# fengranMark/HAConvDR

Hardware: AMD Instinct MI355X
Metric: queries/sec (encode+top-100) over N-passage 768-d corpus; HBM GB/s vs peak (higher is better)
Workload: dtype bf16 MFMA operands with fp32 accumulate / LayerNorm / softmax in the encoder (cosine vs the fp32 reference within 1e-3, measured ~1e-5); search scores and order = the fp32 fmaf chain, bit-exact

## Files before the change

### haconvdr_amd/csrc/encoder.hip

```cpp
#include <type_traits>
#include "hac_common.h"

#include <cmath>
#include <cstring>
#include <map>
#include <string>
#include <vector>

namespace hac {
namespace {

typedef __bf16 bf16;
typedef __bf16 bf16x8 __attribute__((ext_vector_type(8)));
typedef __bf16 bf16x4 __attribute__((ext_vector_type(4)));
typedef float f32x16 __attribute__((ext_vector_type(16)));
typedef float f32x4 __attribute__((ext_vector_type(4)));
typedef float f4v __attribute__((ext_vector_type(4)));

constexpr int H = 768;
constexpr int NH = 12;
constexpr int DH = 64;
constexpr int FF = 3072;
constexpr int SEQ_ALIGN = 32;
constexpr int MT = 256, BK = 64;
// ... 1193 lines not shown
    if (i < n) dst[i] = (bf16)src[i];
}

}
}

using namespace hac;

namespace {

inline int pad_len(int L) { return (L + SEQ_ALIGN - 1) / SEQ_ALIGN * SEQ_ALIGN; }

struct LayerW {
    bf16 *wqkv = nullptr, *wo = nullptr, *w1 = nullptr, *w2 = nullptr;
    float *bqkv = nullptr, *bo = nullptr, *b1 = nullptr, *b2 = nullptr;
    float *ln1g = nullptr, *ln1b = nullptr, *ln2g = nullptr, *ln2b = nullptr;
    bf16 *wqkv8 = nullptr, *w18 = nullptr;
    float *fold = nullptr;
    bf16 *wqkv_lo = nullptr, *wo_lo = nullptr, *w1_lo = nullptr, *w2_lo = nullptr;
};
void free_layer(LayerW &l) {
    for (void *p : std::initializer_list<void *>{l.wqkv, l.wo, l.w1, l.w2, l.wqkv8, l.w18, l.wqkv_lo, l.wo_lo, l.w1_lo, l.w2_lo, l.bqkv, l.fold})
        if (p) (void)hipFree(p);
    l = LayerW();
}
struct Plan {
    const char *gemm = "none";
    int sub_batches = 0;
    long rows = 0;
    const char *graph = "off";
    int precision = 0, pooling = 0, model = 0;
    int ks_out = 1, ks_down = 1;
    int attn_pipe = 0;
};

}

struct hac_encoder {
    hac_encoder_config cfg;
    int device = 0;
    hipStream_t stream = nullptr;
    std::map<std::string, float *> raw;
    std::map<std::string, size_t> raw_count;
    std::vector<LayerW> layers;
    float *word = nullptr, *posw = nullptr, *typew = nullptr, *embg = nullptr, *embb = nullptr;
    float *wh = nullptr, *bh = nullptr, *ng = nullptr, *nb = nullptr;
    bool finalized = false;
    GrowBuf ws_x, ws_xb, ws_q, ws_k, ws_vt, ws_ctx, ws_y, ws_h, ws_seq, ws_ids, ws_mask, ws_out, ws_cls, ws_stats;
    GrowBuf ws_ksplit;
    GrowBuf ws_yb, ws_part, ws_idstats;
    size_t idstats_rows = 0;
    int precision = 0;
    bool split_weights = false;
    int model = 0;
    int pooling = 0;
    GrowBuf ws_pool;
    GrowBuf ws_xb_lo, ws_q_lo, ws_k_lo, ws_vt_lo, ws_ctx_lo, ws_h_lo, ws_cls_lo;
    int attn_mode = 0;
    int attn_pipe = -1;
    int gemm_mode = -1;
    int attn_qsplit = -1;
    int g8_stagger = -1;
    void *h_pin = nullptr;
    size_t h_pin_bytes = 0;
    int *h_len = nullptr;
    size_t h_len_cap = 0;
    unsigned prof_mask = 0;
    struct EvPool {
        std::vector<std::pair<hipEvent_t, hipEvent_t>> ev;
        size_t used = 0;
    } pools[1 + HAC_ENC_NCLASS];
    long max_tokens = 524288;
    int n_cu = 256;
    Plan plan;
    char last_plan[160] = "none";
    int graph_mode = -1;
    int attn_qs_pin = 0;
    int ks_pin_out = 0, ks_pin_down = 0;
    int ksplit_mode = -1;
    struct GraphEntry {
        hipGraph_t graph = nullptr;
        hipGraphExec_t exec = nullptr;
        uint64_t sig = 0;
        int seen = 0;
        Plan plan;
    };
    std::map<uint64_t, GraphEntry> graphs;
    hipEvent_t graph_done = nullptr;
    bool graph_done_armed = false;
    GrowBuf ws_gids, ws_gmask, ws_gout;
    GrowBuf ws_dump;
    GrowBuf ws_identgb;
    GrowBuf ws_redo;
    int *h_redo = nullptr;
    hipEvent_t redo_ev = nullptr;
    bool redo_pending = false;
    long redo_items = 0;
    unsigned pipe_skip_mask = 0;
    unsigned forwards_since_retry = 0;
    GrowBuf ws_clk;
    bool clk_valid = false;
    hipEvent_t clk_ev = nullptr;
};

namespace {

int enc_fail_missing(const std::string &name) { return fail(HAC_ERR_INVALID, "encoder weight '%s' was never set", name.c_str()); }

// ... 101 lines not shown
    };
    for (int i = 0; i < e->cfg.n_layers; ++i) {
        const std::string q = std::string(model_prefix(e)) + "encoder.layer." + std::to_string(i) + ".";
        LayerW &l = e->layers[i];
        float *t;
        if (!l.wqkv_lo) HAC_HIP(hipMalloc((void **)&l.wqkv_lo, (size_t)3 * H * H * sizeof(bf16)));
        if (!l.wo_lo) HAC_HIP(hipMalloc((void **)&l.wo_lo, (size_t)H * H * sizeof(bf16)));
        if (!l.w1_lo) HAC_HIP(hipMalloc((void **)&l.w1_lo, (size_t)FF * H * sizeof(bf16)));
        if (!l.w2_lo) HAC_HIP(hipMalloc((void **)&l.w2_lo, (size_t)H * FF * sizeof(bf16)));
        const char *qkv[3] = {"attention.self.query.weight", "attention.self.key.weight", "attention.self.value.weight"};
        for (int j = 0; j < 3; ++j) {
            HAC_TRY(get_raw(e, q + qkv[j], (size_t)H * H, &t));
            lo(t, (size_t)H * H, l.wqkv_lo + (size_t)j * H * H);
        }
        HAC_TRY(get_raw(e, q + "attention.output.dense.weight", (size_t)H * H, &t));
        lo(t, (size_t)H * H, l.wo_lo);
        HAC_TRY(get_raw(e, q + "intermediate.dense.weight", (size_t)FF * H, &t));
        lo(t, (size_t)FF * H, l.w1_lo);
        HAC_TRY(get_raw(e, q + "output.dense.weight", (size_t)H * FF, &t));
        lo(t, (size_t)H * FF, l.w2_lo);
        HAC_HIP(hipGetLastError());
    }
    HAC_HIP(hipStreamSynchronize(e->stream));
    e->split_weights = true;
    return HAC_OK;
}
int begin_call(hac_encoder *e) {
    e->plan.sub_batches = 0;
    e->plan.rows = 0;
    e->plan.graph = "off";
    e->plan.precision = e->precision;
    e->plan.pooling = e->pooling;
    e->plan.model = e->model;
    return e->precision == 1 ? ensure_split_weights(e) : HAC_OK;
}

struct Fwd {
    int B, L, L32;
    long Mp, Mc;
    SeqInfo s;
    const int *total;
    int family;
    bool big, mean;
    hipStream_t st;
    float *x, *y;
    float2 *statsA, *statsF;
    bf16 *xb, *q, *k, *vt, *ctx, *h;
    bf16 *xb_lo, *q_lo, *k_lo, *vt_lo, *ctx_lo, *h_lo;
    bf16 *yAb;
    float2 *part, *idstats;
    int ks_out, ks_down;
    float *kpart;
    size_t part_stride;
    bf16 *ctx_c, *xb_c, *h_c, *ctx_c_lo, *xb_c_lo, *h_c_lo;
    float *x_c, *y_c, *x2_c;
};

int pick_ksplit(int K, long Mp_plan, long wg_slots, int pin, int ksplit_mode) {
    if (wg_slots == 0 || ksplit_mode == 0) return 1;
    const int KT = K / 64, min_kt = KT >= 48 ? 8 : 4;
    if (pin > 0 && KT % pin == 0 && KT / pin >= 3) return pin;
    const long tiles = (Mp_plan / 128) * (H / 128);
    int S = 1;
    double best = KT * 0.6;
    for (int cand : {2, 3, 4, 6}) {
        if (KT % cand || KT / cand < min_kt || tiles * cand > wg_slots) continue;
// ... 249 lines not shown
int layer_gemm8(hac_encoder *e, const Fwd &f, int li) {
    const LayerW &w = e->layers[li];
    const PrevLN p = prev_ln(e, f, li);
    const hipStream_t st = f.st;
    Gemm8Args a{};
    HAC_TRY(qkv_gemm8(e, f, li, false, a));
    HAC_TRY(attention(e, f, li, false));
    a.A = f.ctx; a.W = w.wo; a.N = H; a.K = H; a.cvec = w.bo; a.resid = f.xb; a.yb = f.yAb; a.part = f.part;
    a.rstats = li ? p.stats : f.idstats;
    a.rgamma = li ? p.g : (const float *)e->ws_identgb.p;
    a.rbeta = li ? p.b : (const float *)e->ws_identgb.p + H;
    a.stagger = stagger8(e, f, H, 0, 8);
    HAC_PROFILED(e, st, HAC_ENC_CLASS_OUTPROJ, launch_gemm8<EPI8_RESID>(e, a, st));
    a.stagger = 0;
    HAC_PROFILED(e, st, HAC_ENC_CLASS_LN, ln_combine_kernel<<<dim3((unsigned)(f.Mp / 256)), dim3(256), 0, st>>>(f.part, H / 64, H, f.total, e->cfg.ln_eps, f.statsA));
    a.A = f.yAb; a.astats = f.statsA; a.W = w.w18; a.N = FF; a.K = H; a.wsum = w.fold + 6 * H; a.cvec = w.fold + 6 * H + FF; a.h = f.h;
    a.n_groups = 2;
    if (e->prof_mask >> 1) {
        HAC_TRY(e->ws_clk.reserve(32));
        a.clk = (unsigned long long *)e->ws_clk.p;
        e->clk_valid = true;
    }
    HAC_TRY(prof_begin(e, 1 + HAC_ENC_CLASS_FFN_UP, st));
    launch_gemm8<EPI8_GELU>(e, a, st);
    if (a.clk) {
        if (!e->clk_ev) HAC_HIP(hipEventCreateWithFlags(&e->clk_ev, hipEventDisableTiming));
        HAC_HIP(hipEventRecord(e->clk_ev, st));
    }
    a.clk = nullptr;
    HAC_TRY(prof_end(e, 1 + HAC_ENC_CLASS_FFN_UP, st));
    a.n_groups = 1;
    a.A = f.h; a.W = w.w2; a.N = H; a.K = FF; a.cvec = w.b2; a.resid = f.yAb; a.yb = f.xb;
    a.rstats = f.statsA; a.rgamma = w.ln1g; a.rbeta = w.ln1b;
    HAC_PROFILED(e, st, HAC_ENC_CLASS_FFN_DOWN, launch_gemm8<EPI8_RESID>(e, a, st));
    HAC_PROFILED(e, st, HAC_ENC_CLASS_LN, ln_combine_kernel<<<dim3((unsigned)(f.Mp / 256)), dim3(256), 0, st>>>(f.part, H / 64, H, f.total, e->cfg.ln_eps, f.statsF));
    return HAC_OK;
}

int tail_classic(hac_encoder *e, const Fwd &f, int li) {
    const LayerW &w = e->layers[li];
    const PrevLN p = prev_ln(e, f, li);
    const hipStream_t st = f.st;
    const bool g8 = f.family == FAM_GEMM8;
    GemmArgs g{};
    Gemm8Args a{};
    HAC_TRY(g8 ? qkv_gemm8(e, f, li, true, a) : qkv_classic(e, f, li, g));
    HAC_TRY(attention(e, f, li, true));
    gather_cls_kernel<<<dim3((unsigned)f.Mc), dim3(256), 0, st>>>(f.ctx, f.x, g8 ? f.xb : nullptr, p.stats, p.g, p.b, f.s, f.B, f.ctx_c, f.x_c);
    g.total_rows = f.s.nb;
    g.A = f.ctx_c; g.W = w.wo; g.bias = w.bo; g.N = H; g.K = H; g.resid = f.x_c; g.y = f.y_c; g.rstats = nullptr;
    launch_gemm128<EPI_RESID>(e, g, st);
    ln_rows_kernel<<<dim3((unsigned)(f.Mc / 4)), dim3(256), 0, st>>>(f.y_c, f.s.nb, w.ln1g, w.ln1b, e->cfg.ln_eps, f.x2_c, f.xb_c);
    g.A = f.xb_c; g.W = w.w1; g.bias = w.b1; g.N = FF; g.K = H; g.h = f.h_c;
    launch_gemm128<EPI_GELU>(e, g, st);
    g.A = f.h_c; g.W = w.w2; g.bias = w.b2; g.N = H; g.K = FF; g.resid = f.x2_c; g.y = f.y_c;
    launch_gemm128<EPI_RESID>(e, g, st);
    ln_rows_kernel<<<dim3((unsigned)(f.Mc / 4)), dim3(256), 0, st>>>(f.y_c, f.s.nb, w.ln2g, w.ln2b, e->cfg.ln_eps, f.x_c, f.xb_c);
    return HAC_OK;
}

template <int EPI>
void launch_gemm_split(const hac_encoder *e, const GemmSplitArgs &ga, hipStream_t st) {
    gemm_split_nt_kernel<EPI><<<dim3((unsigned)e->n_cu), dim3(256), SPLIT_GEMM_LDS, st>>>(ga);
}
int qkv_attention_split(hac_encoder *e, const Fwd &f, int li, bool last, GemmSplitArgs &ga) {
    const LayerW &w = e->layers[li];
    const hipStream_t st = f.st;
// ... 142 lines not shown
    if ((long)B * pad_len(L) > GRAPH_MAX_ROWS || (long)B * pad_len(L) > e->max_tokens) return false;
    hipStreamCaptureStatus cs = hipStreamCaptureStatusNone;
    if (hipStreamIsCapturing(st, &cs) != hipSuccess || cs != hipStreamCaptureStatusNone) return false;
    return true;
}
template <typename IT>
int graph_capture(hac_encoder *e, hac_encoder::GraphEntry &ge, const IT *gids, const IT *gmask, int B, int L, float *gout) {
    if (ge.exec) graphs_quiesce(e);
    if (ge.exec) (void)hipGraphExecDestroy(ge.exec);
    if (ge.graph) (void)hipGraphDestroy(ge.graph);
    ge.exec = nullptr;
    ge.graph = nullptr;
    HAC_HIP(hipStreamSynchronize(e->stream));
    HAC_HIP(hipStreamBeginCapture(e->stream, hipStreamCaptureModeThreadLocal));
    const int rc = run_forward<IT>(e, gids, gmask, B, L, gout, e->stream);
    const hipError_t ce = hipStreamEndCapture(e->stream, &ge.graph);
    if (rc != HAC_OK) return rc;
    if (ce != hipSuccess || !ge.graph) return fail(HAC_ERR_HIP, "hipStreamEndCapture failed: %s", hipGetErrorString(ce));
    HAC_HIP(hipGraphInstantiate(&ge.exec, ge.graph, nullptr, nullptr, 0));
    ge.sig = ws_signature(e);
    ge.plan = e->plan;
    return HAC_OK;
}
template <typename IT>
int forward_graph(hac_encoder *e, const IT *ids, const IT *mask, int B, int L, float *out_dev, hipStream_t st) {
    const size_t n_in = (size_t)B * L * sizeof(IT), n_out = (size_t)B * H * 4;
    HAC_TRY(e->ws_gids.reserve(n_in));
    HAC_TRY(e->ws_gmask.reserve(n_in));
    HAC_TRY(e->ws_gout.reserve(n_out));
    const uint64_t key = ((uint64_t)B << 40) | ((uint64_t)L << 24) | ((uint64_t)sizeof(IT) << 16) | ((uint64_t)(e->attn_mode & 1) << 8) |
                         ((uint64_t)((e->gemm_mode + 1) & 3) << 4) | ((uint64_t)(e->ksplit_mode & 1) << 12) |
                         ((uint64_t)(e->attn_qsplit & 1) << 13) | ((uint64_t)(e->g8_stagger & 1) << 14) | ((uint64_t)((e->attn_pipe + 1) & 3) << 15) |
                         ((uint64_t)(e->precision & 1) << 20) | ((uint64_t)(e->pooling & 1) << 21) |
                         ((uint64_t)(e->model & 1) << 22);
    if (e->graphs.size() >= GRAPH_MAX_SHAPES && e->graphs.find(key) == e->graphs.end()) drop_graphs(e);
    hac_encoder::GraphEntry &ge = e->graphs[key];
    const IT *gids = (const IT *)e->ws_gids.p, *gmask = (const IT *)e->ws_gmask.p;
    float *gout = (float *)e->ws_gout.p;
    HAC_HIP(hipMemcpyAsync(e->ws_gids.p, ids, n_in, hipMemcpyDeviceToDevice, st));
    HAC_HIP(hipMemcpyAsync(e->ws_gmask.p, mask, n_in, hipMemcpyDeviceToDevice, st));
    if (ge.seen == 0) {
        HAC_TRY(run_forward<IT>(e, gids, gmask, B, L, gout, st));
        ge.seen = 1;
        e->plan.graph = "eager-first";
    } else {
        if (!ge.exec || ge.sig != ws_signature(e)) HAC_TRY(graph_capture<IT>(e, ge, gids, gmask, B, L, gout));
        HAC_HIP(hipGraphLaunch(ge.exec, st));
        if (!e->graph_done) HAC_HIP(hipEventCreateWithFlags(&e->graph_done, hipEventDisableTiming));
        HAC_HIP(hipEventRecord(e->graph_done, st));
        e->graph_done_armed = true;
        e->plan = ge.plan;
        e->plan.graph = "replay";
    }
    HAC_HIP(hipMemcpyAsync(out_dev, gout, n_out, hipMemcpyDeviceToDevice, st));
    return HAC_OK;
}

template <typename IT>
int forward_batched(hac_encoder *e, const IT *ids, const IT *mask, int B, int L, float *out_dev, hipStream_t st) {
    const int L32 = pad_len(L);
    HAC_TRY(begin_call(e));
    if (graph_eligible(e, B, L, st)) return forward_graph<IT>(e, ids, mask, B, L, out_dev, st);
    if ((long)B * L32 <= e->max_tokens) return run_forward<IT>(e, ids, mask, B, L, out_dev, st);
    SeqInfo s;
    HAC_TRY(seq_layout(e, B, L, s));
    seq_prep_kernel<IT><<<dim3(B), dim3(512), 0, st>>>(ids, mask, L, s, e->cfg.pad_token_id, e->cfg.vocab, e->model == 1 ? POS_BERT : POS_ROBERTA);
    HAC_HIP(hipGetLastError());
// ... 62 lines not shown
    HAC_HIP(hipMalloc((void **)&l.w18, (size_t)FF * H * sizeof(bf16)));
    HAC_HIP(hipMalloc((void **)&l.fold, (size_t)(2 * 3 * H + 2 * FF) * 4));
    const float *pg = i ? e->layers[i - 1].ln2g : nullptr, *pb = i ? e->layers[i - 1].ln2b : nullptr;
    const float qscale = 0.125f * 1.44269504088896341f;
    for (int j = 0; j < 3; ++j)
        fold_ln_kernel<<<dim3(H), dim3(256), 0, e->stream>>>(ws[j], bs[j], pg, pb, H, j == 0 ? qscale : 1.0f, l.wqkv8 + (size_t)j * H * H,
                                                             l.fold + j * H, l.fold + 3 * H + j * H);
    HAC_TRY(get_raw(e, q + "intermediate.dense.weight", (size_t)FF * H, &t));
    fold_ln_kernel<<<dim3(FF), dim3(256), 0, e->stream>>>(t, l.b1, l.ln1g, l.ln1b, H, 1.0f, l.w18, l.fold + 6 * H, l.fold + 6 * H + FF);
    HAC_HIP(hipGetLastError());
    return HAC_OK;
}

void raise_lds_limits() {
    (void)hipFuncSetAttribute((const void *)attention_kernel<8, 1>, hipFuncAttributeMaxDynamicSharedMemorySize, 65536);
    (void)hipFuncSetAttribute((const void *)attention_kernel<16, 1>, hipFuncAttributeMaxDynamicSharedMemorySize, 131072);
    (void)hipFuncSetAttribute((const void *)attention_stream_kernel<8>, hipFuncAttributeMaxDynamicSharedMemorySize, 81920);
    (void)hipFuncSetAttribute((const void *)attention_stream_kernel<16>, hipFuncAttributeMaxDynamicSharedMemorySize, 163840);
    (void)hipFuncSetAttribute((const void *)attention_pipe_kernel<4>, hipFuncAttributeMaxDynamicSharedMemorySize, 81920);
    (void)hipFuncSetAttribute((const void *)attention_pipe_kernel<8>, hipFuncAttributeMaxDynamicSharedMemorySize, 163840);
    (void)hipFuncSetAttribute((const void *)gemm_bf16_nt_kernel<EPI_QKV, 2>, hipFuncAttributeMaxDynamicSharedMemorySize, 81920);
    (void)hipFuncSetAttribute((const void *)gemm_bf16_nt_kernel<EPI_RESID, 2>, hipFuncAttributeMaxDynamicSharedMemorySize, 81920);
    (void)hipFuncSetAttribute((const void *)gemm_bf16_nt_kernel<EPI_GELU, 2>, hipFuncAttributeMaxDynamicSharedMemorySize, 81920);
    (void)hipFuncSetAttribute((const void *)gemm_bf16_nt_kernel<EPI_QKV, 4>, hipFuncAttributeMaxDynamicSharedMemorySize, 163840);
    (void)hipFuncSetAttribute((const void *)gemm_bf16_nt_kernel<EPI_RESID, 4>, hipFuncAttributeMaxDynamicSharedMemorySize, 163840);
    (void)hipFuncSetAttribute((const void *)gemm_bf16_nt_kernel<EPI_GELU, 4>, hipFuncAttributeMaxDynamicSharedMemorySize, 163840);
    (void)hipFuncSetAttribute((const void *)gemm_split_nt_kernel<EPI_QKV>, hipFuncAttributeMaxDynamicSharedMemorySize, SPLIT_GEMM_LDS);
    (void)hipFuncSetAttribute((const void *)gemm_split_nt_kernel<EPI_RESID>, hipFuncAttributeMaxDynamicSharedMemorySize, SPLIT_GEMM_LDS);
    (void)hipFuncSetAttribute((const void *)gemm_split_nt_kernel<EPI_GELU>, hipFuncAttributeMaxDynamicSharedMemorySize, SPLIT_GEMM_LDS);
    (void)hipFuncSetAttribute((const void *)attention_split_kernel, hipFuncAttributeMaxDynamicSharedMemorySize, 2 * ATS_STAGE);
    (void)hipFuncSetAttribute((const void *)gemm8_kernel<EPI8_QKV, true>, hipFuncAttributeMaxDynamicSharedMemorySize, 163840);
    (void)hipFuncSetAttribute((const void *)gemm8_kernel<EPI8_RESID, false>, hipFuncAttributeMaxDynamicSharedMemorySize, 163840);
    (void)hipFuncSetAttribute((const void *)gemm8_kernel<EPI8_GELU, true>, hipFuncAttributeMaxDynamicSharedMemorySize, 163840);
}

}

extern "C" {

int hac_encoder_create(const hac_encoder_config *cfg, int device, hac_encoder **out) {
    if (!out || !cfg) return fail(HAC_ERR_INVALID, "hac_encoder_create: null argument");
    *out = nullptr;
    if (cfg->hidden != H || cfg->n_heads != NH || cfg->ffn != FF)
        return fail(HAC_ERR_UNSUPPORTED, "only the RoBERTa-base geometry of ANCE is built (hidden 768, 12 heads, ffn 3072); got %d/%d/%d", cfg->hidden,
                    cfg->n_heads, cfg->ffn);
    if (cfg->n_layers < 1 || cfg->n_layers > 48 || cfg->vocab < 1 || cfg->max_pos < 3 || cfg->type_vocab < 1)
        return fail(HAC_ERR_INVALID, "bad encoder config");
    int n_visible = 0;
    if (hipGetDeviceCount(&n_visible) != hipSuccess || n_visible <= 0)
        return fail(HAC_ERR_HIP, "no HIP device visible: the haconvdr encoder has no CPU fallback");
    if (device < 0 || device >= n_visible) return fail(HAC_ERR_INVALID, "device id %d out of range (visible: %d)", device, n_visible);
    hac_encoder *e = new hac_encoder();
    e->cfg = *cfg;
    e->device = device;
    DeviceGuard g(device);
    if (hipStreamCreateWithFlags(&e->stream, hipStreamNonBlocking) != hipSuccess) {
        delete e;
        return fail(HAC_ERR_HIP, "hipStreamCreate failed");
    }
    raise_lds_limits();
    const char *m = getenv("HAC_ENC_GEMM");
    if (m && !parse_gemm_mode(m, &e->gemm_mode)) {
        delete e;
        return fail(HAC_ERR_INVALID, "HAC_ENC_GEMM = '%s': auto | classic | 8phase", m);
    }
    {
// ... 164 lines not shown
    HAC_HIP(hipMemcpy(rows_out, d_rows, nv * 4, hipMemcpyDeviceToHost));
    HAC_HIP(hipMemcpy(stats_out, d_stats, n * 8, hipMemcpyDeviceToHost));
    if (norm_out) HAC_HIP(hipMemcpy(norm_out, d_norm, nv * 4, hipMemcpyDeviceToHost));
    return HAC_OK;
}

int hac_encoder_set_option(hac_encoder *e, const char *name, const char *value) {
    if (!e || !name || !value) return fail(HAC_ERR_INVALID, "set_option: null argument");
    const std::string n(name), v(value);
    if (n == "gemm") {
        if (!parse_gemm_mode(value, &e->gemm_mode)) return fail(HAC_ERR_INVALID, "encoder option gemm = '%s': auto | classic | 8phase", value);
    } else if (n == "precision") {
        if (v != "bf16" && v != "split") return fail(HAC_ERR_INVALID, "encoder option precision = '%s': bf16 | split", value);
        e->precision = v == "split" ? 1 : 0;
    } else if (n == "model") {
        if (v != "roberta" && v != "bert") return fail(HAC_ERR_INVALID, "encoder option model = '%s': roberta | bert", value);
        if (!e->raw.empty()) return fail(HAC_ERR_INVALID, "encoder option model = '%s': must be set before the first hac_encoder_set_weight", value);
        e->model = v == "bert" ? 1 : 0;
    } else if (n == "pooling") {
        if (v != "first" && v != "mean") return fail(HAC_ERR_INVALID, "encoder option pooling = '%s': first | mean", value);
        e->pooling = v == "mean" ? 1 : 0;
    } else if (n == "attn") {
        if (v != "stream" && v != "twopass") return fail(HAC_ERR_INVALID, "encoder option attn = '%s': stream | twopass", value);
        e->attn_mode = v == "twopass" ? 1 : 0;
    } else if (n == "attn_pipe") {
        if (v != "auto" && v != "off" && v != "all") return fail(HAC_ERR_INVALID, "encoder option attn_pipe = '%s': auto | off | all", value);
        e->attn_pipe = v == "off" ? 0 : (v == "all" ? 1 : -1);
    } else if (n == "attn_qsplit") {
        if (v != "auto" && v != "off") return fail(HAC_ERR_INVALID, "encoder option attn_qsplit = '%s': auto | off", value);
        e->attn_qsplit = v == "off" ? 0 : -1;
    } else if (n == "g8_stagger") {
        if (v != "auto" && v != "off") return fail(HAC_ERR_INVALID, "encoder option g8_stagger = '%s': auto | off", value);
        e->g8_stagger = v == "off" ? 0 : -1;
    } else if (n == "attn_qs_pin") {
        if (v != "0" && v != "1" && v != "2" && v != "4" && v != "8" && v != "16") return fail(HAC_ERR_INVALID, "encoder option attn_qs_pin = '%s': 0 | 1 | 2 | 4 | 8 | 16", value);
        e->attn_qs_pin = atoi(v.c_str());
        drop_graphs(e);
    } else if (n == "ksplit_pin") {
        int a = 0, b = 0;
        if (sscanf(v.c_str(), "%d/%d", &a, &b) != 2 || a < 0 || b < 0 || a > 16 || b > 16) return fail(HAC_ERR_INVALID, "encoder option ksplit_pin = '%s': a/b with 0 <= a, b <= 16", value);
        e->ks_pin_out = a;
        e->ks_pin_down = b;
        drop_graphs(e);
    } else if (n == "ksplit") {
        if (v != "auto" && v != "off") return fail(HAC_ERR_INVALID, "encoder option ksplit = '%s': auto | off", value);
        e->ksplit_mode = v == "off" ? 0 : -1;
    } else if (n == "graph") {
        if (v != "auto" && v != "off") return fail(HAC_ERR_INVALID, "encoder option graph = '%s': auto | off", value);
        e->graph_mode = v == "off" ? 0 : -1;
    } else if (n == "max_tokens") {
        char *end = nullptr;
        const long t = strtol(value, &end, 10);
        if (end == value || *end || t < 4096) return fail(HAC_ERR_INVALID, "encoder option max_tokens = '%s': an integer >= 4096", value);
        e->max_tokens = t;
    } else {
        return fail(HAC_ERR_INVALID, "unknown encoder option '%s'", name);
    }
    return HAC_OK;
}

const char *hac_encoder_last_plan(hac_encoder *e) {
    if (!e) return "none";
    const Plan &p = e->plan;
    const bool split = p.precision == 1;
    snprintf(e->last_plan, sizeof e->last_plan, "gemm=%s attn=%s sub_batches=%d rows=%ld graph=%s ksplit=%d/%d attn_form=%s%s%s%s", p.gemm, e->attn_mode ? "twopass" : "stream",
             p.sub_batches, p.rows, p.graph, p.ks_out, p.ks_down,
             split ? "split" : (e->attn_mode ? "twopass" : (p.attn_pipe ? "woven" : "single")), split ? " precision=split" : "", p.pooling == 1 ? " pool=mean" : "", p.model == 1 ? " model=bert" : "");
    return e->last_plan;
}

int hac_encoder_set_profiling(hac_encoder *e, int mask) {
    if (!e) return fail(HAC_ERR_INVALID, "null encoder");
    e->prof_mask = (unsigned)mask & ((2u << HAC_ENC_NCLASS) - 1u);
    return HAC_OK;
}

static int drain_pool(hac_encoder *e, int pool, float *ms_out, int cap, int *n_out) {
    auto &pl = e->pools[pool];
    int n = 0;
    for (size_t i = 0; i < pl.used && n < cap; ++i, ++n) {
        HAC_HIP(hipEventSynchronize(pl.ev[i].second));
        HAC_HIP(hipEventElapsedTime(&ms_out[n], pl.ev[i].first, pl.ev[i].second));
    }
    pl.used = 0;
    *n_out = n;
    return HAC_OK;
}

int hac_encoder_profile_drain(hac_encoder *e, float *ms_out, int cap, int *n_out) {
    if (!e || !n_out || (cap > 0 && !ms_out)) return fail(HAC_ERR_INVALID, "bad arguments");
    DeviceGuard g(e->device);
    return drain_pool(e, 0, ms_out, cap, n_out);
}

int hac_encoder_last_clock(hac_encoder *e, uint64_t out[2]) {
    if (!e || !out) return fail(HAC_ERR_INVALID, "hac_encoder_last_clock: null argument");
    out[0] = out[1] = 0;
    if (!e->clk_valid || !e->ws_clk.p) return HAC_OK;
    DeviceGuard g(e->device);
    unsigned long long h[4] = {0, 0, 0, 0};
// ... 30 lines not shown
```

### haconvdr_amd/csrc/gemm8.inc

```

enum { EPI8_QKV = 0, EPI8_RESID = 2, EPI8_GELU = 3 };
#ifndef G8_N1
#define G8_N1 4
#endif

struct Gemm8Args {
    const bf16 *A;
    const bf16 *W;
    int N, K;
    int n_groups;
    int n_tile0;
    const int *total_rows;
    const float2 *astats;
    const float *wsum;
    const float *cvec;
    bf16 *q, *k, *v16;
    const bf16 *resid;
    const float2 *rstats;
    const float *rgamma, *rbeta;
    bf16 *yb;
    float2 *part;
    bf16 *h;
    unsigned long long *clk;
    int stagger;
    int stagger_mode;
};

__device__ __forceinline__ void glds16(const bf16 *src, unsigned char *dst) {
    typedef const __attribute__((address_space(1))) void *gvp;
    typedef __attribute__((address_space(3))) void *lvp;
    __builtin_amdgcn_global_load_lds((gvp)src, (lvp)dst, 16, 0, 0);
}
__device__ __forceinline__ void swap16(unsigned &a, unsigned &b) {
    const auto r = __builtin_amdgcn_permlane16_swap(a, b, false, false);
// ... 43 lines not shown
typedef unsigned g8_u2 __attribute__((ext_vector_type(2)));
template <bool NT> __device__ __forceinline__ void g8_store16(void *p, uint4 v) {
    if constexpr (NT) __builtin_nontemporal_store(g8_u4{v.x, v.y, v.z, v.w}, reinterpret_cast<g8_u4 *>(p));
    else *reinterpret_cast<uint4 *>(p) = v;
}
template <bool NT> __device__ __forceinline__ void g8_store8(void *p, uint2 v) {
    if constexpr (NT) __builtin_nontemporal_store(g8_u2{v.x, v.y}, reinterpret_cast<g8_u2 *>(p));
    else *reinterpret_cast<uint2 *>(p) = v;
}

__device__ __forceinline__ unsigned pack_bf16(float lo, float hi) {
    typedef __bf16 bf16x2_t __attribute__((ext_vector_type(2)));
    bf16x2_t v;
    v.x = (bf16)lo;
    v.y = (bf16)hi;
    return __builtin_bit_cast(unsigned, v);
}

__device__ __forceinline__ f2v gelu8_2(f2v x) {
    f2v z = x * 0.70710678118654752f;
    z.x = __builtin_amdgcn_fmed3f(z.x, -3.0f, 3.0f);
    z.y = __builtin_amdgcn_fmed3f(z.y, -3.0f, 3.0f);
    const f2v u = z * z;
    f2v p = u * (-1.546677965e-07f) + 6.9032217e-06f;
    p = p * u + (-0.0001336812065f);
    p = p * u + 0.001487465865f;
    p = p * u + (-0.0106578986f);
    p = p * u + 0.0524059485f;
    p = p * u + (-0.1851637965f);
    p = p * u + 0.56346134f;
    return x * (z * p + 0.5f);
}

template <int EPI, bool NT>
__global__ __launch_bounds__(512, 2) void gemm8_kernel(Gemm8Args g) {
    extern __shared__ __attribute__((aligned(16))) unsigned char smem[];
    const int tid = threadIdx.x, lane = tid & 63;
    const int w = __builtin_amdgcn_readfirstlane(tid >> 6);
    const int wr = w >> 2, wc = w & 3;
    if constexpr (EPI == EPI8_GELU) {
        if (g.clk && blockIdx.x == 0 && tid == 0) {
            g.clk[0] = __builtin_amdgcn_s_memtime();
            g.clk[1] = __builtin_amdgcn_s_memrealtime();
        }
    }
    const int K = g.K, KT = K >> 6, nx = (g.N >> 8) - g.n_tile0;
    const int NG = g.n_groups, nxg = nx / NG, NP = 8 / NG;
    const int xcd = blockIdx.x & 7, slot = blockIdx.x >> 3, per_xcd = (gridDim.x + 7 - xcd) >> 3;
    const int mt_all = (*g.total_rows + 255) >> 8;
    const int mt_lo = (int)((long)mt_all * (xcd / NG) / NP), mt_hi = (int)((long)mt_all * (xcd / NG + 1) / NP);
    const int n_base = g.n_tile0 + (xcd % NG) * nxg;
    const int run_lo = 0, run_hi = (mt_hi - mt_lo) * nxg;
    const int tile0 = run_lo + slot;
    if (tile0 >= run_hi) return;
    const int my_tiles = (run_hi - tile0 + per_xcd - 1) / per_xcd;
    const int srow = lane >> 3;
    const int sch0 = (lane & 7) ^ (srow >> 1);
    const int chE = sch0 * 8, chO = (sch0 ^ 4) * 8;
    int s_tile = tile0, s_kt = 0;
    const bf16 *s_A = g.A + (size_t)((mt_lo + s_tile / nxg) << 8) * K, *s_W = g.W + (size_t)((n_base + s_tile % nxg) << 8) * K;
    const int wq = w & 3;
    const int so = EPI == EPI8_RESID ? wr : wr ^ 1;
    const unsigned lsrcE = (unsigned)(((so ? wq * 64 : wq * 32) + srow) * K + chE);
    const unsigned lsrcO = (unsigned)(((so ? wq * 64 : wq * 32) + 8 + srow) * K + chO);
    const int ring_base = (so ? 98304 : 0) + wq * 4096, ring_slots = so ? 4 : 6;
    int h_half = 0, h_slot = 0, h_p = 0;
    const bf16 *h_base = so ? s_W : s_A;
    long h_left = (long)my_tiles * KT * 8;
    constexpr int N1 = G8_N1, N2 = 8 - N1;
    auto issue_piece = [&]() __attribute__((always_inline)) {
        const bf16 *src = h_base + (size_t)(h_half * (so ? 32 : 128) + (h_p >> 1) * 16) * K + s_kt * 64;
        unsigned char *dst = smem + ring_base + (h_slot << 14) + h_p * 1024;
        glds16(src + ((h_p & 1) ? lsrcO : lsrcE), dst);
        if (++h_p == 4) {
            h_p = 0;
            h_slot = h_slot + 1 == ring_slots ? 0 : h_slot + 1;
            if (++h_half == 2) {
                h_half = 0;
                if (++s_kt == KT) {
                    s_kt = 0;
                    s_tile += per_xcd;
                    h_base = so ? g.W + (size_t)((n_base + s_tile % nxg) << 8) * K : g.A + (size_t)((mt_lo + s_tile / nxg) << 8) * K;
                }
            }
        }
    };
    auto issue_pieces = [&](auto ntag) __attribute__((always_inline)) -> bool {
        constexpr int n = decltype(ntag)::value;
        if (h_left <= 0) return false;
        h_left -= n;
#pragma unroll
        for (int i = 0; i < n; ++i) issue_piece();
        return true;
    };
    constexpr std::integral_constant<int, 16> n16tag{};
    constexpr std::integral_constant<int, 8> n8ktag{};

    const int m16 = lane & 15, kg = lane >> 4, sw = (m16 >> 1) & 7;
    const int c0 = ((kg ^ sw) << 4), c1 = (((4 + kg) ^ sw) << 4);
    const int a_row = (wr * 64 + m16) * 128, w_row = (wc * 32 + m16) * 128;

#ifdef G8_STAMP
    unsigned long long stamps[16] = {0, 0, 0, 0, 0, 0, 0, 0, 0, 0, 0, 0, 0, 0, 0, 0};
    unsigned long long est[16] = {0, 0, 0, 0, 0, 0, 0, 0, 0, 0, 0, 0, 0, 0, 0, 0};
#define G8_T(i, cond) if (cond) stamps[i] = __builtin_amdgcn_s_memtime()
#define G8_E(i) if (seq == 2) est[i] = __builtin_amdgcn_s_memtime()
#else
#define G8_E(i)
#define G8_T(i, cond)
#endif
#ifdef G8_STAMP2
    unsigned long long ph[16] = {0, 0, 0, 0, 0, 0, 0, 0, 0, 0, 0, 0, 0, 0, 0, 0};
#define G8_P(i) if (seq == 3 && kt == 6) ph[i] = __builtin_amdgcn_s_memtime()
#define G8_PM() if (seq == 3 && kt == 6) ph[5] = ph[6] = ph[13] = ph[7] = ph[8] = ph[9] = __builtin_amdgcn_s_memtime()
#else
#define G8_P(i)
#define G8_PM()
#endif
    constexpr bool RL = EPI == EPI8_RESID;
    f32x4 acc[2][2][4][2];
    bf16x8 wf0[2][2], wf1[2][2], af0[4][2];

    issue_pieces(n16tag);
    if (g.stagger) {
        const int ph = g.stagger_mode == 0 ? (xcd & 3) : g.stagger_mode == 1 ? (slot & 3) : g.stagger_mode == 2 ? xcd : (slot & 7);
        for (int i = ph * g.stagger; i > 0; --i) __builtin_amdgcn_s_sleep(32);
    }
    asm volatile("s_waitcnt vmcnt(0)" ::: "memory");
    __builtin_amdgcn_s_barrier();

    int a_cur = 0, w_cur = 0;
    for (int seq = 0; seq < my_tiles; ++seq) {
        const int tile = tile0 + seq * per_xcd;
        const int m0 = (mt_lo + tile / nxg) << 8, n0 = (n_base + tile % nxg) << 8;
        unsigned char *R1 = smem, *R2 = smem, *R3 = smem;
        const size_t rl_tb = (size_t)m0 * H + n0;
        auto rl_issue_sb = [&](int i, int mt, unsigned char *dst) __attribute__((always_inline)) {
            int ln = lane;
            asm volatile("" : "+v"(ln));
            const unsigned lo = (unsigned)((ln & 15) * H + (ln >> 5) * 16 + ((ln >> 4) & 1) * 8);
#if defined(G8_RL_ABL) && (G8_RL_ABL & 2)
            const bf16 *src = g.resid + (size_t)(wr * 64 + i * 128 + mt * 16) * H + wc * 64 + lo;
#else
            const bf16 *src = g.resid + (rl_tb + (size_t)(wr * 64 + i * 128 + mt * 16) * H + wc * 64) + lo;
#endif
            glds16(src, dst);
            glds16(src + 32, dst + 1024);
        };
        auto rl_issue_cols = [&](unsigned char *dst) __attribute__((always_inline)) {
            int ln = lane;
            asm volatile("" : "+v"(ln));
            const unsigned so = (unsigned)((ln >> 5) * 128 + 2 * (ln & 31));
// ... 174 lines not shown
            __builtin_amdgcn_sched_barrier(0);
            G8_P(7);
            if (lastk) {
            } else if (kt) {
                if (!live2) asm volatile("s_waitcnt vmcnt(0)" ::: "memory");
                else if (wr == 0) asm volatile("s_waitcnt vmcnt(8)" ::: "memory");
                else asm volatile("s_waitcnt vmcnt(%0)" ::"n"(N2) : "memory");
            }
            asm volatile("s_waitcnt lgkmcnt(0)" ::: "memory");
            G8_P(8);
            __builtin_amdgcn_s_barrier();
            G8_P(9);
            __builtin_amdgcn_sched_barrier(0);
            __builtin_amdgcn_s_setprio(1);
#pragma unroll
            for (int ks = 0; ks < 2; ++ks)
#pragma unroll
                for (int mt = 0; mt < 4; ++mt)
#pragma unroll
                    for (int nt = 0; nt < 2; ++nt) {
                        acc[1][0][mt][nt] = __builtin_amdgcn_mfma_f32_16x16x32_bf16(wf0[nt][ks], af0[mt][ks], acc[1][0][mt][nt], 0, 0, 0);
                        acc[1][1][mt][nt] = __builtin_amdgcn_mfma_f32_16x16x32_bf16(wf1[nt][ks], af0[mt][ks], acc[1][1][mt][nt], 0, 0, 0);
                    }
            __builtin_amdgcn_s_setprio(0);
            G8_P(10);
            __builtin_amdgcn_s_barrier();
            G8_P(11);
            a_cur = a_cur == 2 ? 0 : a_cur + 1;
            w_cur ^= 1;
        }
        G8_T(8, seq == 2 && true);
        if (wr == 0) __builtin_amdgcn_s_barrier();
        G8_T(0, seq == 2);
        if constexpr (!RL) {
            if (wr == 0) issue_pieces(n8ktag);
            asm volatile("s_waitcnt vmcnt(0)" ::: "memory");
        }
        G8_T(1, seq == 2);

#ifdef G8_NO_EPI
#pragma unroll
        for (int i = 0; i < 2; ++i)
#pragma unroll
            for (int j = 0; j < 2; ++j)
#pragma unroll
                for (int mt = 0; mt < 4; ++mt)
#pragma unroll
                    for (int nt = 0; nt < 2; ++nt) asm volatile("" ::"v"(acc[i][j][mt][nt]));
        continue;
#endif
        {
            const int colg = 8 * ((kg & 1) * 2 + (kg >> 1));
            if constexpr (RL) {
                const bool lo8 = m16 < 8;
                const unsigned lane_b = (unsigned)((wr * 64 + (m16 & 7)) * H + wc * 64 + (m16 >> 3) * 32 + colg);
                const unsigned rd_off = (unsigned)(((kg >> 1) * 16 + m16) * 16);
                const bool rd_hi = kg & 1;
#define G8_VM(n) asm volatile("s_waitcnt vmcnt(" #n ")" ::: "memory")
#define G8_VMC(c, a, b) do { if (c) G8_VM(a); else G8_VM(b); } while (0)
#define G8_LDS_DONE() asm volatile("s_waitcnt lgkmcnt(0)" ::: "memory")
                constexpr std::integral_constant<int, -1> cnone{};
                constexpr std::integral_constant<int, 0> c0t{};
                constexpr std::integral_constant<int, 1> c1t{};
                constexpr std::integral_constant<int, 2> c2t{};
                constexpr std::integral_constant<int, 3> c3t{};
                constexpr std::integral_constant<int, 8> n8tag{};
                rl_issue_sb(0, 3, R3);
                rl_issue_sb(1, 0, R3 + 2048);
// ... 98 lines not shown
                G8_VMC(gA, 20, 12);
                G8_E(5);
                sb_do(c0t, c2t, R2 + 2048, c2t, nullptr);
                G8_VMC(gA, 23, 15);
                G8_E(6);
                sb_do(c0t, c3t, R3, c3t, nullptr);
                G8_VMC(gA, 26, 18);
                G8_E(7);
                sb_do(c1t, c0t, R3 + 2048, cnone, nullptr);
                G8_VM(16);
                G8_E(8);
                sb_do(c1t, c1t, R2, cnone, nullptr);
                G8_VM(14);
                G8_E(9);
                sb_do(c1t, c2t, R2 + 2048, cnone, nullptr);
                G8_E(10);
                G8_VM(12);
                G8_E(11);
                g8_u4 c7[2][2];
                sb_read(R3, c7);
                G8_LDS_DONE();
                __builtin_amdgcn_s_barrier();
                if (wr == 1) gW = issue_pieces(n8tag);
                __builtin_amdgcn_sched_barrier(0);
                G8_E(12);
                sb_do(c1t, c3t, R3, cnone, c7);
                G8_E(13);
                G8_VMC(gW, 3, 27);
                G8_E(14);
                G8_E(15);
#undef G8_VM
#undef G8_VMC
#undef G8_LDS_DONE
            } else {
                float2 st[2][4];
#pragma unroll
                for (int i = 0; i < 2; ++i)
#pragma unroll
                    for (int mt = 0; mt < 4; ++mt) st[i][mt] = g.astats[(size_t)m0 + i * 128 + wr * 64 + mt * 16 + m16];
                const int ldo = EPI == EPI8_GELU ? g.N : H;
                const bool lo8 = m16 < 8;
                const unsigned lane_b = (unsigned)((wr * 64 + (m16 & 7)) * ldo + wc * 64 + (m16 >> 3) * 32 + colg);
                f4v ws[2][2], cv[2][2];
#pragma unroll
                for (int j = 0; j < 2; ++j)
#pragma unroll
                    for (int nt = 0; nt < 2; ++nt) {
                        const int nb = n0 + wc * 64 + j * 32;
                        cv[j][nt] = *reinterpret_cast<const f4v *>(g.cvec + nb + nt * 16 + 4 * kg);
                        ws[j][nt] = *reinterpret_cast<const f4v *>(g.wsum + nb + nt * 16 + 4 * kg);
                    }
#pragma unroll
                for (int i = 0; i < 2; ++i)
#pragma unroll
                    for (int mt = 0; mt < 4; ++mt) {
                        const float nm = -st[i][mt].x * st[i][mt].y;
                        float rs = st[i][mt].y;
                        asm volatile("v_mov_b32 %0, %1" : "=v"(rs) : "v"(st[i][mt].y));
                        uint4 o[2];
#pragma unroll
                        for (int j = 0; j < 2; ++j) {
                            const int nb = n0 + wc * 64 + j * 32;
                            unsigned p[4];
#pragma unroll
                            for (int nt = 0; nt < 2; ++nt) {
                                f4v v = acc[i][j][mt][nt] * rs + (ws[j][nt] * nm + cv[j][nt]);
// ... 27 lines not shown
#pragma unroll
                        for (int j = 0; j < 2; ++j) {
                            if constexpr (EPI == EPI8_GELU) {
                                g8_store16<NT>(g.h + ur + (size_t)(j * 8) * ldo + n0 + lane_b, o[j]);
                            } else {
                                bf16 *dst = n0 < H ? g.q + ur + n0 : g.k + ur + (n0 - H);
                                g8_store16<NT>(dst + (size_t)(j * 8) * ldo + lane_b, o[j]);
                            }
                        }
                    }
            }
        }
    }
    if constexpr (EPI == EPI8_GELU) {
        if (g.clk && blockIdx.x == 0 && tid == 0) {
            g.clk[2] = __builtin_amdgcn_s_memtime();
            g.clk[3] = __builtin_amdgcn_s_memrealtime();
        }
    }
#ifdef G8_STAMP2
    if (blockIdx.x == 8 && lane == 0 && (w == 0 || w == 4)) {
        unsigned long long *o = reinterpret_cast<unsigned long long *>(g.part) + 64 + (w ? 16 : 0);
        for (int i = 0; i < 16; ++i) o[i] = ph[i];
    }
#endif
#ifdef G8_STAMP
    if (blockIdx.x == 8 && lane == 0 && (w == 0 || w == 4)) {
        unsigned long long *o = reinterpret_cast<unsigned long long *>(g.part) + (w ? 16 : 0);
        for (int i = 0; i < 16; ++i) o[i] = stamps[i];
        for (int i = 0; i < 16; ++i) o[32 + i] = est[i];
    }
#endif
}

__global__ __launch_bounds__(256) void ln_combine_kernel(const float2 *__restrict__ part, int n_part, int n_cols, const int *__restrict__ total_rows,
                                                         float eps, float2 *__restrict__ stats) {
    const size_t row = (size_t)blockIdx.x * 256 + threadIdx.x;
    if (row >= (size_t)((*total_rows + 255) & ~255)) return;
    float s1 = 0.f, s2 = 0.f;
    if ((n_part & 1) == 0) {
        const float4 *p4 = reinterpret_cast<const float4 *>(part + row * n_part);
        float4 v[8];
        const int n4 = n_part >> 1;
#pragma unroll
        for (int i = 0; i < 8; ++i) v[i] = i < n4 ? p4[i] : make_float4(0.f, 0.f, 0.f, 0.f);
#pragma unroll
        for (int i = 0; i < 8; ++i) {
            s1 += v[i].x + v[i].z;
            s2 += v[i].y + v[i].w;
        }
        for (int i = 16; i < n_part; ++i) {
            const float2 p = part[row * n_part + i];
            s1 += p.x;
            s2 += p.y;
        }
    } else {
        for (int i = 0; i < n_part; ++i) {
            const float2 p = part[row * n_part + i];
            s1 += p.x;
            s2 += p.y;
        }
    }
    const float mean = s1 / n_cols;
    const float var = fmaxf(s2 / n_cols - mean * mean, 0.f);
    stats[row] = make_float2(mean, rsqrtf(var + eps));
}

__global__ __launch_bounds__(256) void fold_ln_kernel(const float *__restrict__ Wf, const float *__restrict__ bias, const float *__restrict__ gamma,
                                                      const float *__restrict__ beta, int K, float scale, bf16 *__restrict__ Wb,
                                                      float *__restrict__ wsum, float *__restrict__ cvec) {
    __shared__ float red[2][4];
    const int n = blockIdx.x, tid = threadIdx.x;
    float s = 0.f, c = 0.f;
    for (int k = tid; k < K; k += 256) {
        const float wv = Wf[(size_t)n * K + k];
        const bf16 wb = (bf16)(wv * (gamma ? gamma[k] : 1.f) * scale);
        Wb[(size_t)n * K + k] = wb;
        s += (float)wb;
        if (beta) c += beta[k] * wv;
    }
    s = wave_sum(s);
    c = wave_sum(c);
    if ((tid & 63) == 0) {
        red[0][tid >> 6] = s;
        red[1][tid >> 6] = c;
    }
    __syncthreads();
    if (tid == 0) {
        wsum[n] = gamma ? (red[0][0] + red[0][1]) + (red[0][2] + red[0][3]) : 0.f;
        cvec[n] = (bias[n] + (red[1][0] + red[1][1]) + (red[1][2] + red[1][3])) * scale;
    }
}

__global__ void fill_identity_stats_kernel(float2 *__restrict__ stats, size_t n) {
    const size_t i = (size_t)blockIdx.x * blockDim.x + threadIdx.x;
    if (i < n) stats[i] = make_float2(0.f, 1.f);
}
```

Baseline: 8308.

## Add FFN-down GEMM variant with residual loads overlapped against main loop tail

Adds a dedicated gemm8_down_kernel, generated by including gemm8.inc twice, for the FFN-down residual GEMM. It loads half of the residual tile, LN stats, bias, gamma and beta before the final vmcnt wait. The epilogue computes those sub-blocks, issues loads for the rest, stores the first half and then finishes the remainder, instead of the interleaved RL epilogue. The aim is to hide residual-load latency in the epilogue, at the cost of more live registers with launch_bounds(512,2). It is on by default, with an option to fall back, and is added to the graph key and plan string.

```diff
diff --git a/haconvdr_amd/csrc/encoder.hip b/haconvdr_amd/csrc/encoder.hip
--- a/haconvdr_amd/csrc/encoder.hip
+++ b/haconvdr_amd/csrc/encoder.hip
@@ -1249,6 +1249,7 @@
     int precision = 0, pooling = 0, model = 0;
     int ks_out = 1, ks_down = 1;
     int attn_pipe = 0;
+    int g8_down = -1;
 };
 
 }
@@ -1278,6 +1279,7 @@
     int gemm_mode = -1;
     int attn_qsplit = -1;
     int g8_stagger = -1;
+    int g8_down = -1;
     void *h_pin = nullptr;
     size_t h_pin_bytes = 0;
     int *h_len = nullptr;
@@ -1290,7 +1292,7 @@
     long max_tokens = 524288;
     int n_cu = 256;
     Plan plan;
-    char last_plan[160] = "none";
+    char last_plan[192] = "none";
     int graph_mode = -1;
     int attn_qs_pin = 0;
     int ks_pin_out = 0, ks_pin_down = 0;
@@ -1458,6 +1460,7 @@
     e->plan.precision = e->precision;
     e->plan.pooling = e->pooling;
     e->plan.model = e->model;
+    e->plan.g8_down = -1;
     return e->precision == 1 ? ensure_split_weights(e) : HAC_OK;
 }
 
@@ -1773,7 +1776,12 @@
     a.n_groups = 1;
     a.A = f.h; a.W = w.w2; a.N = H; a.K = FF; a.cvec = w.b2; a.resid = f.yAb; a.yb = f.xb;
     a.rstats = f.statsA; a.rgamma = w.ln1g; a.rbeta = w.ln1b;
-    HAC_PROFILED(e, st, HAC_ENC_CLASS_FFN_DOWN, launch_gemm8<EPI8_RESID>(e, a, st));
+    if (e->g8_down != 0) {
+        HAC_PROFILED(e, st, HAC_ENC_CLASS_FFN_DOWN, (gemm8_down_kernel<EPI8_RESID, false><<<dim3((unsigned)e->n_cu), dim3(512), 163840, st>>>(a)));
+    } else {
+        HAC_PROFILED(e, st, HAC_ENC_CLASS_FFN_DOWN, launch_gemm8<EPI8_RESID>(e, a, st));
+    }
+    e->plan.g8_down = e->g8_down != 0;
     HAC_PROFILED(e, st, HAC_ENC_CLASS_LN, ln_combine_kernel<<<dim3((unsigned)(f.Mp / 256)), dim3(256), 0, st>>>(f.part, H / 64, H, f.total, e->cfg.ln_eps, f.statsF));
     return HAC_OK;
 }
@@ -1982,7 +1990,7 @@
                          ((uint64_t)((e->gemm_mode + 1) & 3) << 4) | ((uint64_t)(e->ksplit_mode & 1) << 12) |
                          ((uint64_t)(e->attn_qsplit & 1) << 13) | ((uint64_t)(e->g8_stagger & 1) << 14) | ((uint64_t)((e->attn_pipe + 1) & 3) << 15) |
                          ((uint64_t)(e->precision & 1) << 20) | ((uint64_t)(e->pooling & 1) << 21) |
-                         ((uint64_t)(e->model & 1) << 22);
+                         ((uint64_t)(e->model & 1) << 22) | ((uint64_t)(e->g8_down & 1) << 23);
     if (e->graphs.size() >= GRAPH_MAX_SHAPES && e->graphs.find(key) == e->graphs.end()) drop_graphs(e);
     hac_encoder::GraphEntry &ge = e->graphs[key];
     const IT *gids = (const IT *)e->ws_gids.p, *gmask = (const IT *)e->ws_gmask.p;
@@ -2111,6 +2119,7 @@
     (void)hipFuncSetAttribute((const void *)gemm8_kernel<EPI8_QKV, true>, hipFuncAttributeMaxDynamicSharedMemorySize, 163840);
     (void)hipFuncSetAttribute((const void *)gemm8_kernel<EPI8_RESID, false>, hipFuncAttributeMaxDynamicSharedMemorySize, 163840);
     (void)hipFuncSetAttribute((const void *)gemm8_kernel<EPI8_GELU, true>, hipFuncAttributeMaxDynamicSharedMemorySize, 163840);
+    (void)hipFuncSetAttribute((const void *)gemm8_down_kernel<EPI8_RESID, false>, hipFuncAttributeMaxDynamicSharedMemorySize, 163840);
 }
 
 }
@@ -2341,6 +2350,9 @@
     } else if (n == "g8_stagger") {
         if (v != "auto" && v != "off") return fail(HAC_ERR_INVALID, "encoder option g8_stagger = '%s': auto | off", value);
         e->g8_stagger = v == "off" ? 0 : -1;
+    } else if (n == "g8_down") {
+        if (v != "auto" && v != "one_phase" && v != "two_phase") return fail(HAC_ERR_INVALID, "encoder option g8_down = '%s': auto | one_phase | two_phase", value);
+        e->g8_down = v == "auto" ? -1 : v == "one_phase";
     } else if (n == "attn_qs_pin") {
         if (v != "0" && v != "1" && v != "2" && v != "4" && v != "8" && v != "16") return fail(HAC_ERR_INVALID, "encoder option attn_qs_pin = '%s': 0 | 1 | 2 | 4 | 8 | 16", value);
         e->attn_qs_pin = atoi(v.c_str());
@@ -2372,9 +2384,10 @@
     if (!e) return "none";
     const Plan &p = e->plan;
     const bool split = p.precision == 1;
-    snprintf(e->last_plan, sizeof e->last_plan, "gemm=%s attn=%s sub_batches=%d rows=%ld graph=%s ksplit=%d/%d attn_form=%s%s%s%s", p.gemm, e->attn_mode ? "twopass" : "stream",
+    snprintf(e->last_plan, sizeof e->last_plan, "gemm=%s attn=%s sub_batches=%d rows=%ld graph=%s ksplit=%d/%d attn_form=%s%s%s%s%s", p.gemm, e->attn_mode ? "twopass" : "stream",
              p.sub_batches, p.rows, p.graph, p.ks_out, p.ks_down,
-             split ? "split" : (e->attn_mode ? "twopass" : (p.attn_pipe ? "woven" : "single")), split ? " precision=split" : "", p.pooling == 1 ? " pool=mean" : "", p.model == 1 ? " model=bert" : "");
+             split ? "split" : (e->attn_mode ? "twopass" : (p.attn_pipe ? "woven" : "single")), split ? " precision=split" : "", p.pooling == 1 ? " pool=mean" : "", p.model == 1 ? " model=bert" : "",
+             p.g8_down < 0 ? "" : (p.g8_down ? " g8_down=one_phase" : " g8_down=two_phase"));
     return e->last_plan;
 }
 
diff --git a/haconvdr_amd/csrc/gemm8.inc b/haconvdr_amd/csrc/gemm8.inc
--- a/haconvdr_amd/csrc/gemm8.inc
+++ b/haconvdr_amd/csrc/gemm8.inc
@@ -1,5 +1,7 @@
+#ifndef G8_FORM
 
 enum { EPI8_QKV = 0, EPI8_RESID = 2, EPI8_GELU = 3 };
+#define G8_DA 4
 #ifndef G8_N1
 #define G8_N1 4
 #endif
@@ -109,8 +111,23 @@
     return x * (z * p + 0.5f);
 }
 
+#define G8_FORM 1
+#include "gemm8.inc"
+#undef G8_FORM
+#define G8_FORM 2
+#include "gemm8.inc"
+#undef G8_FORM
+#else
+
 template <int EPI, bool NT>
+#if G8_FORM == 1
 __global__ __launch_bounds__(512, 2) void gemm8_kernel(Gemm8Args g) {
+    constexpr bool DOWN = false;
+#else
+__global__ __launch_bounds__(512, 2) void gemm8_down_kernel(Gemm8Args g) {
+    constexpr bool DOWN = true;
+    static_assert(EPI == EPI8_RESID && !NT, "the FFN-down form of the residual GEMM");
+#endif
     extern __shared__ __attribute__((aligned(16))) unsigned char smem[];
     const int tid = threadIdx.x, lane = tid & 63;
     const int w = __builtin_amdgcn_readfirstlane(tid >> 6);
@@ -137,7 +154,8 @@
     int s_tile = tile0, s_kt = 0;
     const bf16 *s_A = g.A + (size_t)((mt_lo + s_tile / nxg) << 8) * K, *s_W = g.W + (size_t)((n_base + s_tile % nxg) << 8) * K;
     const int wq = w & 3;
-    const int so = EPI == EPI8_RESID ? wr : wr ^ 1;
+    constexpr bool RL = EPI == EPI8_RESID && !DOWN;
+    const int so = RL ? wr : wr ^ 1;
     const unsigned lsrcE = (unsigned)(((so ? wq * 64 : wq * 32) + srow) * K + chE);
     const unsigned lsrcO = (unsigned)(((so ? wq * 64 : wq * 32) + 8 + srow) * K + chO);
     const int ring_base = (so ? 98304 : 0) + wq * 4096, ring_slots = so ? 4 : 6;
@@ -194,7 +212,6 @@
 #define G8_P(i)
 #define G8_PM()
 #endif
-    constexpr bool RL = EPI == EPI8_RESID;
     f32x4 acc[2][2][4][2];
     bf16x8 wf0[2][2], wf1[2][2], af0[4][2];
 
@@ -435,8 +452,37 @@
         G8_T(8, seq == 2 && true);
         if (wr == 0) __builtin_amdgcn_s_barrier();
         G8_T(0, seq == 2);
+        uint4 d_res[2][4][2];
+        float2 d_st[2][4];
+        f4v d_cv[2][2], d_rg[2][2], d_rb[2][2];
+        auto down_load = [&](int sb) __attribute__((always_inline)) {
+            const int i = sb >> 2, mt = sb & 3;
+            int ln = lane;
+            asm volatile("" : "+v"(ln));
+            const int lm = ln & 15, lg = ln >> 4;
+            d_st[i][mt] = g.rstats[(size_t)m0 + i * 128 + wr * 64 + mt * 16 + lm];
+            const unsigned d_lane = (unsigned)((wr * 64 + (lm & 7)) * H + wc * 64 + (lm >> 3) * 32 + 8 * ((lg & 1) * 2 + (lg >> 1)));
+#pragma unroll
+            for (int jj = 0; jj < 2; ++jj)
+                d_res[i][mt][jj] = *reinterpret_cast<const uint4 *>(g.resid + rl_tb + (size_t)((i * 128 + mt * 16 + jj * 8) * H) + d_lane);
+        };
         if constexpr (!RL) {
             if (wr == 0) issue_pieces(n8ktag);
+            if constexpr (DOWN) {
+                __builtin_amdgcn_sched_barrier(0);
+#pragma unroll
+                for (int sb = 0; sb < G8_DA; ++sb) down_load(sb);
+#pragma unroll
+                for (int j = 0; j < 2; ++j)
+#pragma unroll
+                    for (int nt = 0; nt < 2; ++nt) {
+                        const int co = n0 + wc * 64 + j * 32 + nt * 16 + 4 * kg;
+                        d_cv[j][nt] = *reinterpret_cast<const f4v *>(g.cvec + co);
+                        d_rg[j][nt] = *reinterpret_cast<const f4v *>(g.rgamma + co);
+                        d_rb[j][nt] = *reinterpret_cast<const f4v *>(g.rbeta + co);
+                    }
+                __builtin_amdgcn_sched_barrier(0);
+            }
             asm volatile("s_waitcnt vmcnt(0)" ::: "memory");
         }
         G8_T(1, seq == 2);
@@ -601,6 +647,82 @@
 #undef G8_VM
 #undef G8_VMC
 #undef G8_LDS_DONE
+            } else if constexpr (DOWN) {
+                const bool lo8 = m16 < 8;
+                const unsigned lane_b = (unsigned)((wr * 64 + (m16 & 7)) * H + wc * 64 + (m16 >> 3) * 32 + colg);
+#pragma unroll
+                for (int jj = 0; jj < 2; ++jj)
+#pragma unroll
+                    for (int nt = 0; nt < 2; ++nt)
+#pragma unroll
+                        for (int i = 0; i < 2; ++i)
+#pragma unroll
+                            for (int mt = 0; mt < 4; ++mt) acc[i][jj][mt][nt] += d_cv[jj][nt];
+                __builtin_amdgcn_sched_barrier(0);
+                auto sb_compute = [&](int sb, uint4 (&ro)[2], float2 &pt) __attribute__((always_inline)) {
+                    const int i = sb >> 2, mt = sb & 3;
+                    float mean, rstd;
+                    asm volatile("v_mov_b32 %0, %1" : "=v"(mean) : "v"(d_st[i][mt].x));
+                    asm volatile("v_mov_b32 %0, %1" : "=v"(rstd) : "v"(d_st[i][mt].y));
+                    xchg8(d_res[i][mt][0], d_res[i][mt][1], lo8);
+                    float s1 = 0.f, s2 = 0.f;
+#pragma unroll
+                    for (int jj = 0; jj < 2; ++jj) {
+                        unsigned q0 = d_res[i][mt][jj].x, q1 = d_res[i][mt][jj].y, q2 = d_res[i][mt][jj].z, q3 = d_res[i][mt][jj].w;
+                        swap16(q0, q2);
+                        swap16(q1, q3);
+                        const uint2 w0 = {q0, q1}, w1 = {q2, q3};
+                        const f4v ra = {__uint_as_float(w0.x << 16), __uint_as_float(w0.x & 0xffff0000u), __uint_as_float(w0.y << 16), __uint_as_float(w0.y & 0xffff0000u)};
+                        const f4v rb_ = {__uint_as_float(w1.x << 16), __uint_as_float(w1.x & 0xffff0000u), __uint_as_float(w1.y << 16), __uint_as_float(w1.y & 0xffff0000u)};
+                        const f4v o0 = acc[i][jj][mt][0] + ((ra - mean) * rstd * d_rg[jj][0] + d_rb[jj][0]);
+                        const f4v o1 = acc[i][jj][mt][1] + ((rb_ - mean) * rstd * d_rg[jj][1] + d_rb[jj][1]);
+                        unsigned p0 = pack_bf16(o0.x, o0.y), p1 = pack_bf16(o0.z, o0.w);
+                        unsigned p2 = pack_bf16(o1.x, o1.y), p3 = pack_bf16(o1.z, o1.w);
+                        swap16(p0, p2);
+                        swap16(p1, p3);
+                        ro[jj] = make_uint4(p0, p1, p2, p3);
+                        const f4v sm = o0 + o1, sq = o0 * o0 + o1 * o1;
+                        const float t1 = (sm.x + sm.y) + (sm.z + sm.w), t2 = (sq.x + sq.y) + (sq.z + sq.w);
+                        s1 = jj ? s1 + t1 : t1;
+                        s2 = jj ? s2 + t2 : t2;
+                    }
+                    s1 += __shfl_xor(s1, 16);
+                    s2 += __shfl_xor(s2, 16);
+                    s1 += __shfl_xor(s1, 32);
+                    s2 += __shfl_xor(s2, 32);
+                    pt = make_float2(s1, s2);
+                    xchg8(ro[0], ro[1], lo8);
+                    __builtin_amdgcn_sched_barrier(0);
+                };
+                auto sb_store = [&](int sb, const uint4 (&ro)[2], float2 pt) __attribute__((always_inline)) {
+                    const int i = sb >> 2, mt = sb & 3;
+                    int ln = lane;
+                    asm volatile("" : "+v"(ln));
+                    const size_t row = (size_t)m0 + i * 128 + wr * 64 + mt * 16 + (ln & 15);
+                    if (kg == 0) g.part[row * (g.N >> 6) + (n0 >> 6) + wc] = pt;
+#pragma unroll
+                    for (int jj = 0; jj < 2; ++jj)
+                        g8_store16<NT>(g.yb + rl_tb + (size_t)((i * 128 + mt * 16 + jj * 8) * H) + lane_b, ro[jj]);
+                    __builtin_amdgcn_sched_barrier(0);
+                };
+                uint4 ro_h[G8_DA][2];
+                float2 pt_h[G8_DA];
+#pragma unroll
+                for (int sb = 0; sb < G8_DA; ++sb) sb_compute(sb, ro_h[sb], pt_h[sb]);
+#pragma unroll
+                for (int sb = G8_DA; sb < 8; ++sb) down_load(sb);
+                __builtin_amdgcn_sched_barrier(0);
+#pragma unroll
+                for (int sb = 0; sb < G8_DA; ++sb) sb_store(sb, ro_h[sb], pt_h[sb]);
+                static_assert(G8_DA == 4, "the counted wait below");
+                asm volatile("s_waitcnt vmcnt(12)" ::: "memory");
+#pragma unroll
+                for (int sb = G8_DA; sb < 8; ++sb) {
+                    uint4 ro[2];
+                    float2 pt;
+                    sb_compute(sb, ro, pt);
+                    sb_store(sb, ro, pt);
+                }
             } else {
                 float2 st[2][4];
 #pragma unroll
@@ -694,6 +816,8 @@
     }
 #endif
 }
+#endif
+#ifndef G8_FORM
 
 __global__ __launch_bounds__(256) void ln_combine_kernel(const float2 *__restrict__ part, int n_part, int n_cols, const int *__restrict__ total_rows,
                                                          float eps, float2 *__restrict__ stats) {
@@ -758,3 +882,4 @@
     const size_t i = (size_t)blockIdx.x * blockDim.x + threadIdx.x;
     if (i < n) stats[i] = make_float2(0.f, 1.f);
 }
+#endif
```

Result: no change. 8359 (median of 6 runs) (+0.6%).
